# lowmee/xchu_slam

Hardware: AMD Instinct MI355X
Metric: NDT scans/sec (120k-pt scan vs 200k-voxel localmap, 30 iters) at 1/2/4/8 GPUs; % HBM BW (higher is better)
Workload: dtype f32 (f64 accumulate)

## Files before the change

### xchu_slam_amd/csrc/host_sort.hip

```cpp
#include "ndt_host.h"

namespace ndt::host {

ndt_status scan_ctx(ndt_ctx* c, Lane L, int nb, ScanCtx* sc) {
    sc->tickets = c->opt.tile_tickets ? 1 : 0;
    if ((size_t)nb > L.s.scan_status.cap) {
        TRY(ensure(c, L.s.scan_status, (size_t)nb));
        HIPCHK(c, hipMemsetAsync(L.s.scan_status.p, 0, L.s.scan_status.cap * sizeof(unsigned long long), L.st));
    }
    if (!L.s.scan_ticket.p) {
        TRY(ensure(c, L.s.scan_ticket, 1));
        HIPCHK(c, hipMemsetAsync(L.s.scan_ticket.p, 0, sizeof(unsigned long long), L.st));
        L.s.scan_tickets = 0;
    }
    sc->status = L.s.scan_status.p;
    sc->ticket = L.s.scan_ticket.p;
    sc->ticket_base = L.s.scan_tickets;
    sc->epoch = ++L.s.scan_epoch;
    sc->nb = nb;
    if (sc->tickets) L.s.scan_tickets += (unsigned long long)nb;
    return NDT_OK;
}

ndt_status enqueue_scan(ndt_ctx* c, Lane L, const int* in, int n_host, const int* n_dev, int* out, int* total_out, GridHeader* herr) {
    const int nb = std::max(1, ceil_div(n_host, kTileKeys));
    ScanCtx sc;
    TRY(scan_ctx(c, L, nb, &sc));
    hipLaunchKernelGGL(k_scan_onepass, dim3(nb), dim3(kBlock), 0, L.st, in, n_host, n_dev, out, total_out, sc, herr);
    return NDT_OK;
}

constexpr int kRadixWideKeys = 4 << 20;
int radix_items(const ndt_ctx* c, int n) {
    return ceil_div(n, kTileKeys) < c->n_cu ? 4 : (n >= kRadixWideKeys ? 24 : 16);
}
size_t radix_status_words(int nb) { return (size_t)4 * 256 * ((size_t)nb + (size_t)ceil_div(nb, 16)); }
void launch_radix_pass(const ndt_ctx* c, Lane L, int items, int nb, int* k0, int* v0, int* k1, int* v1, int n, int pass,
                       const GridHeader* h, GridHeader* herr, int last_pass) {
    auto* kern = items == 4 ? k_radix_onesweep<4> : items == 16 ? k_radix_onesweep<16> : k_radix_onesweep<24>;
    hipLaunchKernelGGL(kern, dim3(nb), dim3(kBlock), 0, L.st, k0, v0, k1, v1, n, pass, h, L.s.radix_aux.p, L.s.radix_status.p, nb,
                       herr, last_pass, c->opt.tile_tickets ? 1 : 0);
}

int radix_launch_passes(const ndt_ctx* c) {
    if (c->rerun_full) return 4;
    return c->opt.radix_force > 0 ? std::min(c->opt.radix_force, 4) : c->radix_pred;
}
void note_grid_width(ndt_ctx* c, long long cells, int dense) {
    if (cells <= 0) return;
    const long long top = dense ? cells - 1 : cells;
    int bits = 0;
    while (bits < 31 && (top >> bits) != 0) ++bits;
    c->radix_pred = std::min(4, std::max(1, (bits + 1 + 7) / 8));
}

ndt_status enqueue_bin_and_sort(ndt_ctx* c, Lane L, const float4* pts, int n, int dense, GridHeader* h, float leaf, int layout,
                                int binning, int2* cloud_span, int passes) {
    if (&L.s == &c->s && !cloud_span) c->inc_ok = false;
    const int nb_mm = std::max(1, std::min(ceil_div(n, 4 * kBlock), 1024));
    TRY(ensure(c, L.s.mm, (size_t)nb_mm * 7));
    const int items = radix_items(c, n);
    const int nb_sort = std::max(1, ceil_div(n, kBlock * items));
    const size_t n_kv = cloud_span ? (size_t)n + (size_t)n / 4 : (size_t)n;
    TRY(ensure(c, L.s.k0, n_kv)); TRY(ensure(c, L.s.v0, n_kv)); TRY(ensure(c, L.s.k1, n_kv)); TRY(ensure(c, L.s.v1, n_kv));
    TRY(ensure(c, L.s.radix_aux, kRadixAuxWords));
    TRY(ensure(c, L.s.radix_status, radix_status_words(nb_sort)));
    TRY(ensure(c, L.s.seg_start, (size_t)n + 1));
    hipLaunchKernelGGL(k_minmax, dim3(nb_mm), dim3(kBlock), 0, L.st, pts, n, dense, L.s.mm.p, L.s.radix_aux.p,
                       cloud_span ? c->d_clk.p + 3 : nullptr, nullptr, nullptr, nullptr);
    const int nb_keys = std::max(1, std::min(ceil_div(n, 4 * kBlock), 512));
    hipLaunchKernelGGL(k_keys, dim3(nb_keys), dim3(kBlock), 0, L.st, pts, n, dense, L.s.mm.p, nb_mm, h, leaf, c->prm.min_points_per_voxel,
                       c->prm.min_covar_eigvalue_mult, layout, binning, L.s.k0.p, L.s.v0.p, L.s.radix_aux.p, L.s.radix_status.p,
                       (int)radix_status_words(nb_sort), cloud_span ? c->grid.p : nullptr, (long long)c->grid.cap, cloud_span ? c->table.p : nullptr,
                       1LL << c->max_log2cap, nullptr, 0);
    for (int pass = 0; pass < passes; ++pass)
        launch_radix_pass(c, L, items, nb_sort, L.s.k0.p, L.s.v0.p, L.s.k1.p, L.s.v1.p, n, pass, h, h, passes - 1);
    const int nb_seg = std::max(1, ceil_div(n, kTileKeys));
    ScanCtx sc;
    TRY(scan_ctx(c, L, nb_seg, &sc));
    hipLaunchKernelGGL(k_seg_scan, dim3(nb_seg), dim3(kBlock), 0, L.st, L.s.k0.p, L.s.k1.p, n, h, L.s.seg_start.p, sc);
    if (cloud_span) {
        ScanCtx sc2;
        TRY(scan_ctx(c, L, nb_seg, &sc2));
        hipLaunchKernelGGL(k_cloud_scan, dim3(nb_seg), dim3(kBlock), 0, L.st, L.s.seg_start.p, n, h, cloud_span, sc2, c->max_log2cap);
    }
    return NDT_OK;
}

ndt_status enqueue_downsample_finalize(ndt_ctx* c, Lane L, const GridHeader* h, const float4* in, int n, float4* out) {
    TRY(ensure(c, L.s.sorted_pts, std::max(n, 1)));
    const int nb = std::max(1, std::min(ceil_div(n, 4 * kBlock), 2048));
    hipLaunchKernelGGL(k_sorted_gather, dim3(nb), dim3(kBlock), 0, L.st, in, L.s.v0.p, L.s.v1.p, h, L.s.sorted_pts.p, n);
    hipLaunchKernelGGL(k_downsample_finalize, dim3(std::max(1, ceil_div(n, kBlock))), dim3(kBlock), 0, L.st, L.s.sorted_pts.p,
                       L.s.seg_start.p, h, out);
    HIPCHK(c, hipGetLastError());
    return NDT_OK;
}

}
```

### xchu_slam_amd/csrc/host_target.hip

```cpp
#include "ndt_host.h"

namespace ndt::host {

namespace {

ndt_status grow_grid(ndt_ctx* c) {
    const long long want_cells = std::min<long long>(std::max<long long>(2 * c->grid_cells_seen, 16ll << 20), 1ll << 30);
    if ((long long)c->grid.cap < want_cells) TRY(ensure(c, c->grid, (size_t)want_cells));
    return NDT_OK;
}

ndt_status alloc_cloud_buffers(ndt_ctx* c, size_t max_cloud) {
    TRY(ensure(c, c->recs, max_cloud)); TRY(ensure(c, c->cent, max_cloud)); TRY(ensure(c, c->icovd, max_cloud * 9));
    TRY(ensure(c, c->evals, max_cloud * 3)); TRY(ensure(c, c->cloud_key, max_cloud));
    return NDT_OK;
}

constexpr int kFinalize3WavesMaxPoints = 4 << 20;

ndt_status prepare_target_buffers(ndt_ctx* c, int M, int* nb_cloud) {
    TRY(grow_grid(c));
    const size_t max_cloud = std::max(1, M / std::max(1, c->prm.min_points_per_voxel) + 1);
    TRY(alloc_cloud_buffers(c, max_cloud));
    unsigned l = 6;
// ... 9 lines not shown
ndt_status launch_finalize(ndt_ctx* c, int M, int nb_cloud) {
    auto* fin = M < kFinalize3WavesMaxPoints ? k_leaf_finalize<3> : k_leaf_finalize<2>;
    hipLaunchKernelGGL(fin, dim3(nb_cloud), dim3(kBlock), 0, c->stream.get(), c->target_ptr, c->s.k0.p, c->s.k1.p, c->s.v0.p,
                       c->s.v1.p, c->s.cloud_span.p, c->d_hdr.p, c->recs.p, c->cent.p, c->icovd.p, c->cloud_key.p,
                       c->evals.p, c->grid.p, c->table.p, c->valid_part.p);
    HIPCHK(c, hipGetLastError());
    return NDT_OK;
}

ndt_status enqueue_target_build(ndt_ctx* c) {
    c->inc_ok = false;
    ++c->n_builds_full;
    const int M = c->M;
    int nb_cloud = 0;
    TRY(prepare_target_buffers(c, M, &nb_cloud));
    TRY(enqueue_bin_and_sort(c, main_lane(c), c->target_ptr, M, c->target_dense, c->d_hdr.p, c->prm.resolution, 0, c->prm.precision_mode == 2 ? 1 : 0,
                             c->s.cloud_span.p, radix_launch_passes(c)));
    TRY(launch_finalize(c, M, nb_cloud));
    c->inc_ok = c->prm.precision_mode != 2 && c->target_dense == 1 && M > 0;
    return NDT_OK;
}

ndt_status enqueue_target_append(ndt_ctx* c, int n_old, int n_new, const float4* new_src) {
    const int M = n_old + n_new;
    int nb_cloud = 0;
    TRY(prepare_target_buffers(c, M, &nb_cloud));
    Lane Q{c->stream.get(), c->s_inc};
    float4* copy_to = new_src ? const_cast<float4*>(c->target_ptr) + n_old : nullptr;
    const float4* pts_new = new_src ? new_src : c->target_ptr + n_old;
    const int nq = std::max(n_new, 1);
    const int nb_mm = std::max(1, std::min(ceil_div(nq, 4 * kBlock), 1024));
    TRY(ensure(c, Q.s.mm, (size_t)nb_mm * 7));
    const int items = radix_items(c, nq);
    const int nb_sort = std::max(1, ceil_div(nq, kBlock * items));
    TRY(ensure(c, Q.s.k0, nq)); TRY(ensure(c, Q.s.v0, nq)); TRY(ensure(c, Q.s.k1, nq)); TRY(ensure(c, Q.s.v1, nq));
    TRY(ensure(c, Q.s.radix_aux, kRadixAuxWords));
    TRY(ensure(c, Q.s.radix_status, radix_status_words(nb_sort)));
    TRY(ensure(c, c->s.seg_start, (size_t)M + 1));
    hipLaunchKernelGGL(k_minmax, dim3(nb_mm), dim3(kBlock), 0, c->stream.get(), pts_new, n_new, 1, Q.s.mm.p, Q.s.radix_aux.p, c->d_clk.p + 3,
                       c->d_hdr.p, c->d_hdr_prev.p, copy_to);
    if (c->tgt_ev_valid) HIPCHK(c, hipEventRecord(c->ev_tgt.get(), c->stream.get()));
    const long long clear_words = std::max<long long>((long long)c->grid.cap, 2LL << c->max_log2cap) / 4;
    const int nb_keys = std::max(1, (int)std::min<long long>(std::max<long long>(ceil_div(nq, 4 * kBlock), ceil_div(clear_words, 4LL * kBlock)), 512));
    hipLaunchKernelGGL(k_keys, dim3(nb_keys), dim3(kBlock), 0, c->stream.get(), pts_new, n_new, 1, Q.s.mm.p, nb_mm, c->d_hdr.p, c->prm.resolution,
                       c->prm.min_points_per_voxel, c->prm.min_covar_eigvalue_mult, 0, 0, Q.s.k0.p, Q.s.v0.p, Q.s.radix_aux.p,
                       Q.s.radix_status.p, (int)radix_status_words(nb_sort), c->grid.p, (long long)c->grid.cap, c->table.p, 1LL << c->max_log2cap,
                       c->d_hdr_prev.p, n_old);
    const int passes = radix_launch_passes(c);
    for (int pass = 0; pass < passes; ++pass)
        launch_radix_pass(c, Q, items, nb_sort, Q.s.k0.p, Q.s.v0.p, Q.s.k1.p, Q.s.v1.p, n_new, pass, c->d_hdr.p, c->d_hdr.p, passes - 1);
    hipLaunchKernelGGL(k_merge_append, dim3(std::max(1, ceil_div(M, kMergeTileKeys))), dim3(kBlock), 0, c->stream.get(), c->s.k0.p, c->s.v0.p,
                       c->s.k1.p, c->s.v1.p, c->d_hdr_prev.p, n_old, Q.s.k0.p, Q.s.v0.p, Q.s.k1.p, Q.s.v1.p, n_new, c->d_hdr.p,
                       c->target_ptr);
    const Lane L = main_lane(c);
    const int nb_seg = std::max(1, ceil_div(M, kTileKeys));
    ScanCtx sc, sc2;
    TRY(scan_ctx(c, L, nb_seg, &sc));
    hipLaunchKernelGGL(k_seg_scan, dim3(nb_seg), dim3(kBlock), 0, c->stream.get(), c->s.k0.p, c->s.k1.p, M, c->d_hdr.p, c->s.seg_start.p, sc);
    TRY(scan_ctx(c, L, nb_seg, &sc2));
    hipLaunchKernelGGL(k_cloud_scan, dim3(nb_seg), dim3(kBlock), 0, c->stream.get(), c->s.seg_start.p, M, c->d_hdr.p, c->s.cloud_span.p, sc2,
                       c->max_log2cap);
    TRY(launch_finalize(c, M, nb_cloud));
    return NDT_OK;
}

}

ndt_status build_target(ndt_ctx* c) {
    ++c->tgt_gen;
    c->tgt_ev_valid = c->lanes.fit_tgt_used;
    if (c->tgt_ev_valid) HIPCHK(c, hipEventRecord(c->ev_tgt.get(), c->stream.get()));
    TRY(enqueue_target_build(c));
    c->build_unchecked = true;
    c->built_since_align = true;
    c->grid_valid = true;
    c->fit_valid = false;
    c->grid_res = c->prm.resolution;
    c->have_result = false;
    return NDT_OK;
}

ndt_status rerun_build(ndt_ctx* c, int berr) {
    ++c->n_builds_rerun;
    if (berr & kBuildErrLookback) {
        c->opt.tile_tickets = true;
        ++c->n_rerun_lookback;
    }
    c->inc_ok = false;
    c->rerun_full = true;
    const ndt_status st = build_target(c);
    c->rerun_full = false;
    return st;
}

ndt_status settle_build(ndt_ctx* c) {
    if (!c->build_unchecked || !c->grid_valid) return NDT_OK;
    for (int attempt = 0;; ++attempt) {
        HIPCHK(c, hipMemcpyAsync(c->h_hdr.get(), c->d_hdr.p, sizeof(GridHeader), hipMemcpyDeviceToHost, c->stream.get()));
        HIPCHK(c, hipStreamSynchronize(c->stream.get()));
        const int berr = c->h_hdr->pad[0];
        if (!berr) break;
        if (attempt > 0) return fail(c, NDT_EDEVICE, "target build failed twice (error bits " + std::to_string(berr) + ")");
        TRY(rerun_build(c, berr));
    }
    c->build_unchecked = false;
    note_grid_width(c, c->h_hdr->cells, c->target_dense);
    return NDT_OK;
}

ndt_status upload_points(ndt_ctx* c, DevBuf<float4>& dst, const float* xyz, size_t n, size_t stride_bytes) {
    TRY(ensure(c, dst, n));
    std::vector<float4> tmp(n);
    const char* base = reinterpret_cast<const char*>(xyz);
    for (size_t i = 0; i < n; ++i) {
// ... 165 lines not shown
```

### xchu_slam_amd/csrc/ndt_host.h

```cpp
#pragma once
#include <hip/hip_runtime.h>
#include <string>
#include <vector>
#include <cstring>
#include <cstdlib>
#include <cstdio>
#include <algorithm>
#include <cmath>
#include <atomic>
#include <condition_variable>
#include <deque>
#include <functional>
#include <memory>
#include <mutex>
#include <shared_mutex>
#include <thread>

#include "../../include/ndt_hip.h"
#include "ndt_kernels.h"
#include "ndt_geom.h"

namespace ndt::host {

constexpr int kTileKeys = kBlock * 16;
// ... 310 lines not shown

#define TRY(expr)                          \
    do {                                   \
        ndt_status _s = (expr);            \
        if (_s != NDT_OK) return _s;       \
    } while (0)

template <typename T> ndt_status make_pinned(ndt_ctx* c, Pinned<T>& out, size_t n, unsigned flags) {
    void* p = nullptr;
    if (hipHostMalloc(&p, n * sizeof(std::remove_extent_t<T>), flags) != hipSuccess) return fail(c, NDT_ENOMEM, "hipHostMalloc failed");
    out.reset(static_cast<std::remove_extent_t<T>*>(p));
    return NDT_OK;
}
inline ndt_status make_event(ndt_ctx* c, Event& out, unsigned flags) {
    hipEvent_t e = nullptr;
    HIPCHK(c, hipEventCreateWithFlags(&e, flags));
    out.reset(e);
    return NDT_OK;
}
inline ndt_status make_stream(ndt_ctx* c, Stream& out, int priority) {
    hipStream_t st = nullptr;
    HIPCHK(c, hipStreamCreateWithPriority(&st, hipStreamNonBlocking, priority));
    out.reset(st);
    return NDT_OK;
}

inline void hand_options(ndt_ctx* h, const ndt_ctx* c) {
    const bool sticky = h->opt.tile_tickets;
    h->opt = c->opt;
    h->opt.tile_tickets = sticky || c->opt.tile_tickets;
}

inline ndt_status set_dev(ndt_ctx* c) {
    HIPCHK(c, hipSetDevice(c->device));
    return NDT_OK;
}

inline ndt_status need_target_and_source(ndt_ctx* c) {
    if (!c->has_target) return fail(c, NDT_ENOTARGET, "no input target");
    if (!c->has_source || c->N == 0) return fail(c, NDT_ENOSOURCE, "no input source");
    return NDT_OK;
}

ndt_status scan_ctx(ndt_ctx* c, Lane L, int nb, ScanCtx* sc);
ndt_status enqueue_scan(ndt_ctx* c, Lane L, const int* in, int n_host, const int* n_dev, int* out, int* total_out, GridHeader* herr);
int radix_items(const ndt_ctx* c, int n);
size_t radix_status_words(int nb);
void launch_radix_pass(const ndt_ctx* c, Lane L, int items, int nb, int* k0, int* v0, int* k1, int* v1, int n, int pass,
                       const GridHeader* h, GridHeader* herr, int last_pass = 3);
int radix_launch_passes(const ndt_ctx* c);
void note_grid_width(ndt_ctx* c, long long cells, int dense);
ndt_status enqueue_bin_and_sort(ndt_ctx* c, Lane L, const float4* pts, int n, int dense, GridHeader* h, float leaf, int layout = 0,
                                int binning = 0, int2* cloud_span = nullptr, int passes = 4);
ndt_status enqueue_downsample_finalize(ndt_ctx* c, Lane L, const GridHeader* h, const float4* in, int n, float4* out);
ndt_status build_target(ndt_ctx* c);
ndt_status rerun_build(ndt_ctx* c, int berr);
ndt_status settle_build(ndt_ctx* c);
ndt_status upload_points(ndt_ctx* c, DevBuf<float4>& dst, const float* xyz, size_t n, size_t stride_bytes);
void invalidate_graph(ndt_ctx* c);
ndt_status copy16(ndt_ctx* c, hipStream_t stream, void* dst, const void* src, size_t bytes);
ndt_status flush_source(ndt_ctx* c);
ndt_status capture_graph(ndt_ctx* c, const char* end_what, const std::function<ndt_status()>& body, GraphExec* out);
ndt_status main_after_fit(ndt_ctx* c, bool source);
ndt_status enqueue_nn_index(ndt_ctx* c, Lane L, const float4* pts, int n, int dense, float cell, NNIndex& ix, bool want_idx = false);
ndt_status ensure_fit_index(ndt_ctx* c);
ndt_status voxel_downsample_dev(ndt_ctx* c, const float4* in, size_t n, float leaf, float4* out, size_t* n_out);
ndt_status reserve_slots(ndt_ctx* c, SlotArrays& a, size_t size, size_t need, std::initializer_list<size_t> slot_bytes, const char* what);

}
```

### xchu_slam_amd/csrc/ndt_kernels.h

```cpp
#pragma once
#include <hip/hip_runtime.h>
#include "ndt_types.h"
#include "ndt_linalg.h"
#include "ndt_icp.h"
#include "ndt_sc.h"
#include "ndt_isc.h"
#include "ndt_pgo.h"
#include "ndt_map.h"

namespace ndt {
__global__ void k_minmax(const float4*, int, int, float*, int*, unsigned long long*, const GridHeader*, GridHeader*, float4*);
__global__ void k_keys(const float4*, int, int, const float*, int, GridHeader*, float, int, double, int, int, int*, int*, int*, unsigned*, int,
                       int*, long long, int2*, long long, const GridHeader*, int);
__global__ void k_merge_append(int*, int*, int*, int*, const GridHeader*, int, const int*, const int*, const int*, const int*, int,
                               GridHeader*, const float4*);
template <int ITEMS>
__global__ void k_radix_onesweep(int*, int*, int*, int*, int, int, const GridHeader*, int*, unsigned*, int, GridHeader*, int, int);
__global__ void k_scan_onepass(const int*, int, const int*, int*, int*, ScanCtx, GridHeader*);
__global__ void k_seg_scan(const int*, const int*, int, GridHeader*, int*, ScanCtx);
__global__ void k_cloud_scan(const int*, int, GridHeader*, int2*, ScanCtx, unsigned);

template <int WAVES>
__global__ void k_leaf_finalize(const float4*, const int*, const int*, const int*, const int*, const int2*, GridHeader*,
                                VoxelRec*, float4*, double*, int*, double*, int*, int2*, int*);
__global__ void k_sorted_gather(const float4*, const int*, const int*, const GridHeader*, float4*, int);
__global__ void k_src_keys(const float4*, int, Mat4f, const GridHeader*, int*, int*, int*, unsigned*, int);
__global__ void k_src_gather(const float4*, const int*, const int*, const GridHeader*, float4*, int);
__global__ void k_crop_flags(const float4*, int, double, double, int*);
__global__ void k_compact4(const float4*, const int*, const int*, int, float4*);
template <int C>
__global__ void k_sor_knn(const float4*, int, int, const GridHeader*, const int*, const int*, const float4*, float*);
__global__ void k_sor_stats(const float*, int, double, double*);
__global__ void k_sor_keep(const float*, int, const double*, int*);
__global__ void k_ror_keep(const float4*, int, double, int, const GridHeader*, const int*, const int*, const float4*, int*);
__global__ void k_downsample_finalize(const float4*, const int*, const GridHeader*, float4*);
__global__ void k_fit_gather(const float4*, const int*, const int*, const int*, const int*, const int*, int, const GridHeader*, float4*,
                             int*, int*, int*);
__global__ void k_icp_pass(float4*, int, IcpState*, const GridHeader*, const int*, const int*, const float4*, const int*, int*, float*,
                           double*, unsigned*, IcpRecordDev*);
__global__ void k_sc_make(const float4*, int, unsigned*);
__global__ void k_sc_finalize(const unsigned*, ScDb, int);
__global__ void k_sc_detect(ScDb, const int*, const int*, int, int, ScDetectArgs, ndt_sc_result*);
__global__ void k_isc_make(const float4*, int, IscGeom, unsigned*);
__global__ void k_isc_finalize(const unsigned*, IscDb, int, int, int, double, double, double, double);
__global__ void k_isc_detect(IscDb, const int*, int, IscDetectArgs, IscPartial*);
__global__ void k_isc_reduce(const IscPartial*, const int*, int, int, IscDetectArgs, ndt_isc_result*);
__global__ void k_pgo_optimize(PgoGraph, PgoArgs);
__global__ void k_map_stack(const float4*, const int*, const long long*, const Mat4f*, int, int, int, float4*);
__global__ void k_fit_block_flags(const int*, const GridHeader*, int*);
__global__ void k_append2(const float4*, const float4*, int, const GridHeader*, float4*, float4*);
__global__ void k_fit_block_clear(int*, const GridHeader*);
__global__ void k_fit_tables(const int*, const int*, const int*, const int*, const GridHeader*, int*, int*);
__global__ void k_fitness(const float4*, int, Mat4f, const GridHeader*, const int*, const int*, const float4*, double, float*, double*,
                          int*, unsigned*, double*, long long*);
__global__ void k_score_radius(const float4*, int, Mat4f, const GridHeader*, const int2*, const int*, const VoxelRec*, const float4*,
                               const double*, double, double, double, float, double*);
template <int SEARCH, int PPT, bool ONE_TILE>
__global__ void k_pass_direct(const float4*, int, int, const GridHeader*, const int2*, const int*, const VoxelRec*, const AlignState*,
                              AlignState*, double*, unsigned*, double*, PassRecordDev*, int, int, unsigned long long*, int4*);
__global__ void k_pass_radius(const float4*, int, const GridHeader*, const int2*, const int*, const VoxelRec*, const float4*,
                              const double*, const AlignState*, AlignState*, double*, unsigned*, double*, PassRecordDev*, int, int,
                              unsigned long long*);
__global__ void k_transform(const float4*, int, const AlignState*, float4*);
__global__ void k_transform_mat(const float4*, int, Mat4f, float4*);
__global__ void k_align_init(const AlignState, AlignState*, unsigned*, unsigned long long*, int, unsigned long long*, const GridHeader*,
                             unsigned long long, const uint4*, uint4*, long long);
__global__ void k_copy16(const uint4*, uint4*, size_t);
__global__ void k_readback(const unsigned long long*, unsigned long long*, int, const unsigned long long*, unsigned long long*, int,
                           const unsigned long long*, unsigned long long*, int, const unsigned long long*, unsigned long long*,
                           unsigned long long*, unsigned long long, unsigned long long*, const GridHeader*);
hipError_t dbg_read_blk(unsigned long long* host, size_t count);
__global__ void k_svd_resume(AlignState*);
template <int SEARCH, bool ONE_TILE>
// ... 4 lines not shown
```

### xchu_slam_amd/csrc/voxel_build.hip

```cpp
#include "ndt_device.h"
#include "ndt_kernels.h"

namespace ndt {

constexpr int kTileItems = 16;
constexpr int kTile = kBlock * kTileItems;
constexpr int kRadixAux = kRadixAuxWords;

__global__ __launch_bounds__(kBlock) void k_minmax(const float4* __restrict__ pts, int n, int is_dense, float* __restrict__ part,
                                                   int* __restrict__ radix_aux, unsigned long long* __restrict__ clk_start,
                                                   const GridHeader* __restrict__ hdr_cur, GridHeader* __restrict__ hdr_save,
                                                   float4* __restrict__ copy_to) {
    if (clk_start && blockIdx.x == 0 && threadIdx.x == 0) *clk_start = __builtin_amdgcn_s_memrealtime();
    if (blockIdx.x == 0) {
        for (int i = threadIdx.x; i < kRadixAux; i += kBlock) radix_aux[i] = 0;
        if (hdr_save) {
            static_assert(sizeof(GridHeader) % 4 == 0 && sizeof(GridHeader) / 4 <= kBlock, "header copy: one word per thread");
            if (threadIdx.x < sizeof(GridHeader) / 4)
                reinterpret_cast<int*>(hdr_save)[threadIdx.x] = reinterpret_cast<const int*>(hdr_cur)[threadIdx.x];
        }
    }
    float mn[3] = {FLT_MAX, FLT_MAX, FLT_MAX}, mx[3] = {-FLT_MAX, -FLT_MAX, -FLT_MAX};
    int cnt = 0;
    const int stride = gridDim.x * kBlock;
// ... 483 lines not shown
__device__ __forceinline__ int scan_n(int n, const int* n_dev) { return n_dev ? *n_dev : n; }

__device__ __forceinline__ const int* sorted_buf_nominal(const GridHeader* h, const int* b0, const int* b1) {
    const int passes = (h->key_bits + 7) / 8;
    return (passes & 1) ? b1 : b0;
}
__device__ __forceinline__ const int* sorted_buf(const GridHeader* h, const int* b0, const int* b1) {
    const int passes = (h->key_bits + 7) / 8;
    return ((passes + h->flip) & 1) ? b1 : b0;
}

constexpr unsigned long long kScanAgg = 1ull << 30, kScanPre = 2ull << 30, kScanVal = (1ull << 30) - 1;

__device__ long long scan_lookback(unsigned long long* __restrict__ status, int tile, int tot, unsigned epoch,
                                   GridHeader* __restrict__ herr) {
    const int lane = threadIdx.x & 63;
    const unsigned long long tag = (unsigned long long)epoch << 32;
    if (lane == 0)
        __hip_atomic_store(&status[tile], tag | (tile == 0 ? kScanPre : kScanAgg) | (unsigned long long)tot, __ATOMIC_RELAXED,
                           __HIP_MEMORY_SCOPE_AGENT);
    long long excl = 0;
    int t = tile - 1;
    int spin = 0;
    while (t >= 0) {
        const int tt = t - lane;
        unsigned long long wd = 0;
        bool ready = true;
        if (tt >= 0) {
            wd = __hip_atomic_load(&status[tt], __ATOMIC_RELAXED, __HIP_MEMORY_SCOPE_AGENT);
            ready = (wd >> 32) == epoch && (wd & (kScanAgg | kScanPre)) != 0;
        }
        const bool pre = tt >= 0 && ready && (wd & kScanPre);
        const unsigned long long pre_mask = __ballot(pre);
        const int stop = pre_mask ? (__ffsll((long long)pre_mask) - 1) : 63;
        const unsigned long long need = (stop == 63) ? ~0ull : ((2ull << stop) - 1);
        const unsigned long long not_ready = __ballot(!ready) & need;
        if (not_ready) {
            if (++spin > kSpinLimit) { if (lane == 0) atomicOr(&herr->pad[0], kBuildErrLookback); break; }
            __builtin_amdgcn_s_sleep(1);
            continue;
        }
        long long v = (tt >= 0 && lane <= stop) ? (long long)(wd & kScanVal) : 0;
        for (int m = 32; m > 0; m >>= 1) v += __shfl_xor(v, m, 64);
        excl += v;
        if (pre_mask) break;
        t -= 64;
    }
    if (lane == 0 && tile > 0)
        __hip_atomic_store(&status[tile], tag | kScanPre | ((unsigned long long)(excl + tot) & kScanVal), __ATOMIC_RELAXED,
                           __HIP_MEMORY_SCOPE_AGENT);
    return excl;
}

__device__ __forceinline__ int tile_scan(const ScanCtx& sc, int sum, GridHeader* herr, int* s_tile, int* s_excl, int* lds, int tile,
                                         int* total) {
    int tot;
    const int ex = block_exclusive_scan(sum, lds, &tot);
    if (threadIdx.x < 64) {
        const long long excl = scan_lookback(sc.status, tile, tot, sc.epoch, herr);
        if (threadIdx.x == 0) *s_excl = (int)excl;
    }
    __syncthreads();
    *total = *s_excl + tot;
    return ex + *s_excl;
}

__device__ __forceinline__ int take_ticket(const ScanCtx& sc, int* s_tile) {
    if (threadIdx.x == 0) *s_tile = sc.tickets ? (int)(atomicAdd(sc.ticket, 1ull) - sc.ticket_base) : (int)blockIdx.x;
    __syncthreads();
    return *s_tile;
}

constexpr int kStageWords = kTile + 2 + (kTile + 2) / 32 + 1;
__host__ __device__ constexpr int st_idx(int p) { return p + (p >> 5); }
template <int EXTRA>
__device__ __forceinline__ void stage_tile(const int* __restrict__ in, long long first, int n, int fill, int* s) {
    constexpr int R = (kTile + EXTRA + kBlock - 1) / kBlock;
    int v[R];
#pragma unroll
    for (int r = 0; r < R; ++r) {
        const int p = threadIdx.x + r * kBlock;
        const long long i = first + p;
        v[r] = (p < kTile + EXTRA && i >= 0 && i < n) ? in[i] : fill;
    }
#pragma unroll
    for (int r = 0; r < R; ++r) {
        const int p = threadIdx.x + r * kBlock;
        if (p < kTile + EXTRA) s[st_idx(p)] = v[r];
    }
    __syncthreads();
}

__global__ __launch_bounds__(kBlock) void k_scan_onepass(const int* __restrict__ in, int n, const int* n_dev, int* __restrict__ out,
                                                         int* __restrict__ total_out, ScanCtx sc, GridHeader* __restrict__ herr) {
    __shared__ int s_tile, s_excl, lds[4];
    __shared__ int s_in[kStageWords];
    const int tile = take_ticket(sc, &s_tile);
    const int nn = scan_n(n, n_dev);
    const int base = tile * kTile + threadIdx.x * kTileItems;
    stage_tile<0>(in, (long long)tile * kTile, nn, 0, s_in);
    int loc[kTileItems];
    int sum = 0;
#pragma unroll
    for (int k = 0; k < kTileItems; ++k) {
        loc[k] = s_in[st_idx(threadIdx.x * kTileItems + k)];
        sum += loc[k];
    }
    int total;
    int ex = tile_scan(sc, sum, herr, &s_tile, &s_excl, lds, tile, &total);
    if (tile == sc.nb - 1 && threadIdx.x == 0 && total_out) *total_out = total;
#pragma unroll
    for (int k = 0; k < kTileItems; ++k) {
        if (base + k < nn) out[base + k] = ex;
        ex += loc[k];
    }
// ... 61 lines not shown
            const unsigned long long probed = __ballot(m < hi);
            const unsigned long long fls = __ballot(m < hi && !t);
            if (fls == 0ull) {
                lo = lo + (63 - __clzll((long long)probed)) * step + 1;
            } else {
                const int f = __ffsll((long long)fls) - 1;
                const int nlo = f == 0 ? lo : lo + (f - 1) * step + 1;
                hi = lo + f * step;
                lo = nlo;
            }
        }
        if (lane == 0) s_split[w] = lo;
    }
    __syncthreads();
    const int a0 = s_split[0], a1 = s_split[1];
    const int la = a1 - a0, b0 = d0 - a0, lb = (d1 - d0) - la;
    for (int i = threadIdx.x; i < la; i += kBlock) {
        const int v = ov[a0 + i];
        s_k[i] = remap_key(r, ok[a0 + i], v, pts, hn);
        s_v[i] = v;
    }
    for (int i = threadIdx.x; i < lb; i += kBlock) {
        s_k[la + i] = qk[b0 + i];
        s_v[la + i] = qv[b0 + i];
    }
    __syncthreads();
    const int dl = threadIdx.x * kMergeItems;
    const int tn = d1 - d0;
    if (dl >= tn) return;
    int lo = max(0, dl - lb), hi = min(dl, la);
    while (lo < hi) {
        const int mid = (lo + hi) >> 1;
        if (s_k[mid] <= s_k[la + dl - 1 - mid]) lo = mid + 1;
        else hi = mid;
    }
    int ai = lo, bi = dl - lo;
#pragma unroll
    for (int k = 0; k < kMergeItems; ++k) {
        if (dl + k >= tn) break;
        const bool take_a = ai < la && (bi >= lb || s_k[ai] <= s_k[la + bi]);
        const int src = take_a ? ai : la + bi;
        wk[d0 + dl + k] = s_k[src];
        wv[d0 + dl + k] = s_v[src];
        ai += take_a ? 1 : 0;
        bi += take_a ? 0 : 1;
    }
}

__global__ __launch_bounds__(kBlock) void k_seg_scan(const int* __restrict__ k0, const int* __restrict__ k1, int n,
                                                     GridHeader* __restrict__ h, int* __restrict__ seg_start, ScanCtx sc) {
    __shared__ int s_tile, s_excl, lds[4];
    __shared__ int s_k[kStageWords];
    const int tile = take_ticket(sc, &s_tile);
    const bool empty = h->empty != 0;
    const int* k = sorted_buf(h, k0, k1);
    const int sentinel = h->sentinel;
    const int base = tile * kTile + threadIdx.x * kTileItems;
    unsigned heads = 0;
    int sum = 0;
    if (!empty) {
        stage_tile<1>(k, (long long)tile * kTile - 1, n, 0, s_k);
        int prev = s_k[st_idx(threadIdx.x * kTileItems)];
#pragma unroll
        for (int q = 0; q < kTileItems; ++q) {
            const int i = base + q;
            if (i >= n) break;
            const int key = s_k[st_idx(threadIdx.x * kTileItems + q + 1)];
            if (key != sentinel && (i == 0 || prev != key)) { heads |= 1u << q; ++sum; }
            prev = key;
        }
    }
    int total;
    int ex = tile_scan(sc, sum, h, &s_tile, &s_excl, lds, tile, &total);
#pragma unroll
    for (int q = 0; q < kTileItems; ++q)
        if (heads & (1u << q)) seg_start[ex++] = base + q;
    if (tile == sc.nb - 1 && threadIdx.x == 0) {
        h->n_leaves = total;
        seg_start[total] = empty ? 0 : h->n_points;
    }
}

__global__ __launch_bounds__(kBlock) void k_cloud_scan(const int* __restrict__ seg_start, int n, GridHeader* __restrict__ h,
                                                       int2* __restrict__ cloud_span, ScanCtx sc, unsigned max_log2cap) {
    __shared__ int s_tile, s_excl, lds[4];
    __shared__ int s_seg[kStageWords];
    const int tile = take_ticket(sc, &s_tile);
    const int nl = h->empty ? 0 : h->n_leaves;
    const int last = nl > 0 ? (nl - 1) / kTile : 0;
    if (tile > last) return;
    const int base = tile * kTile + threadIdx.x * kTileItems;
    const int minp = h->min_points;
    unsigned fl = 0;
    int sum = 0;
    stage_tile<1>(seg_start, (long long)tile * kTile, nl + 1, 0, s_seg);
#pragma unroll
    for (int q = 0; q < kTileItems; ++q) {
        const int s = base + q;
        if (s >= nl) break;
        const int p = threadIdx.x * kTileItems + q;
        if (s_seg[st_idx(p + 1)] - s_seg[st_idx(p)] >= minp) { fl |= 1u << q; ++sum; }
    }
    int total;
    int ex = tile_scan(sc, sum, h, &s_tile, &s_excl, lds, tile, &total);
#pragma unroll
    for (int q = 0; q < kTileItems; ++q)
        if (fl & (1u << q)) {
            const int p = threadIdx.x * kTileItems + q;
            cloud_span[ex++] = make_int2(s_seg[st_idx(p)], s_seg[st_idx(p + 1)]);
        }
    if (tile == last && threadIdx.x == 0) {
        h->n_cloud = total;
        unsigned l = 6;
        while (l < max_log2cap && (1LL << l) < 4LL * (long long)total) ++l;
        h->log2cap = l;
        if (total == 0) h->empty = 1;
    }
}






constexpr int kGather = 8;
__device__ __forceinline__ bool leaf_stats(const float4* __restrict__ pts, const int* __restrict__ idx, int b, int e, int ci, int key,
                                           const GridHeader* __restrict__ h, VoxelRec* __restrict__ recs, float4* __restrict__ cent,
                                           double* __restrict__ icovd, int* __restrict__ cloud_key, double* __restrict__ evals_out) {
    const int n = e - b;
    double sum[3] = {0.0, 0.0, 0.0};
    double cov[9] = {1.0, 0.0, 0.0, 0.0, 1.0, 0.0, 0.0, 0.0, 1.0};
    float cen[3] = {0.f, 0.f, 0.f};
    int ix[kGather];
#pragma unroll
    for (int k = 0; k < kGather; ++k) ix[k] = (b + k < e) ? idx[b + k] : -1;
    for (int j0 = b; j0 < e; j0 += kGather) {
        float4 q[kGather];
#pragma unroll
        for (int k = 0; k < kGather; ++k) q[k] = ix[k] >= 0 ? pts[ix[k]] : make_float4(0.f, 0.f, 0.f, 0.f);
#pragma unroll
        for (int k = 0; k < kGather; ++k) ix[k] = (j0 + kGather + k < e) ? idx[j0 + kGather + k] : -1;
#pragma unroll
        for (int k = 0; k < kGather; ++k) {
            if (j0 + k >= e) break;
            const float4 p = q[k];
            const double pd[3] = {(double)p.x, (double)p.y, (double)p.z};
            sum[0] += pd[0]; sum[1] += pd[1]; sum[2] += pd[2];
            for (int c = 0; c < 3; ++c)
                for (int r = 0; r < 3; ++r) cov[r + 3 * c] += pd[r] * pd[c];
            cen[0] += p.x; cen[1] += p.y; cen[2] += p.z;
        }
    }
    const float nf = (float)n;
    for (int a = 0; a < 3; ++a) cen[a] /= nf;
    const double nd = (double)n;
    double mean[3];
    for (int a = 0; a < 3; ++a) mean[a] = sum[a] / nd;
    if (h->binning)
        for (int a = 0; a < 3; ++a) cen[a] = (float)mean[a];
    for (int c = 0; c < 3; ++c)
        for (int r = 0; r < 3; ++r) cov[r + 3 * c] = (cov[r + 3 * c] - 2 * (sum[r] * mean[c])) / nd + mean[r] * mean[c];
    const double f = (n - 1.0) / n;
    for (int k = 0; k < 9; ++k) cov[k] *= f;
    double ev[3], V[9];
    if (h->binning) aw_sym_eigen3(cov, ev, V);
    else sym_eigen3(cov, ev, V);
    double icov[9] = {0, 0, 0, 0, 0, 0, 0, 0, 0};
    bool rejected = false;
    if (ev[0] < 0 || ev[1] < 0 || ev[2] <= 0) {
        rejected = true;
// ... 448 lines not shown
        s_cnt[threadIdx.x] = k;
        __syncthreads();
        for (int off = kFitBlock / 2; off > 0; off >>= 1) {
            if ((int)threadIdx.x < off) { s_sum[threadIdx.x] += s_sum[threadIdx.x + off]; s_cnt[threadIdx.x] += s_cnt[threadIdx.x + off]; }
            __syncthreads();
        }
    };
    tree(sum, cnt);
    const int nb = gridDim.x;
    const int g = blockIdx.x / kFitGroup, ng = (nb + kFitGroup - 1) / kFitGroup;
    const int g0 = g * kFitGroup, gsize = min(kFitGroup, nb - g0);
    if (threadIdx.x == 0) {
        __hip_atomic_store(part_sum + blockIdx.x, s_sum[0], __ATOMIC_RELAXED, __HIP_MEMORY_SCOPE_AGENT);
        __hip_atomic_store(part_cnt + blockIdx.x, (int)s_cnt[0], __ATOMIC_RELAXED, __HIP_MEMORY_SCOPE_AGENT);
        asm volatile("s_waitcnt vmcnt(0)" ::: "memory");
        s_role = __hip_atomic_fetch_add(&ticket[kFitTicketStride * (1 + g)], 1u, __ATOMIC_RELAXED, __HIP_MEMORY_SCOPE_AGENT) ==
                 (unsigned)gsize - 1;
    }
    __syncthreads();
    if (!s_role) return;
    __builtin_amdgcn_fence(__ATOMIC_ACQUIRE, "agent");
    asm volatile("s_waitcnt vmcnt(0)" ::: "memory");
    {
        const int t = threadIdx.x;
        tree(t < gsize ? part_sum[g0 + t] : 0.0, t < gsize ? (long long)part_cnt[g0 + t] : 0ll);
    }
    if (threadIdx.x == 0) {
        ticket[kFitTicketStride * (1 + g)] = 0u;
        __hip_atomic_store(part_sum + nb + g, s_sum[0], __ATOMIC_RELAXED, __HIP_MEMORY_SCOPE_AGENT);
        __hip_atomic_store(part_cnt + nb + g, (int)s_cnt[0], __ATOMIC_RELAXED, __HIP_MEMORY_SCOPE_AGENT);
        asm volatile("s_waitcnt vmcnt(0)" ::: "memory");
        s_role = __hip_atomic_fetch_add(&ticket[0], 1u, __ATOMIC_RELAXED, __HIP_MEMORY_SCOPE_AGENT) == (unsigned)ng - 1 ? 2 : 0;
    }
    __syncthreads();
    if (s_role != 2) return;
    __builtin_amdgcn_fence(__ATOMIC_ACQUIRE, "agent");
    asm volatile("s_waitcnt vmcnt(0)" ::: "memory");
    {
        double v = 0.0;
        long long k = 0;
        for (int t = threadIdx.x; t < ng; t += kFitBlock) { v += part_sum[nb + t]; k += part_cnt[nb + t]; }
        tree(v, k);
    }
    if (threadIdx.x == 0) {
        __hip_atomic_store(out_sum, s_sum[0], __ATOMIC_RELAXED, __HIP_MEMORY_SCOPE_SYSTEM);
        __hip_atomic_store(out_cnt, h->pad[0] ? -1ll : (long long)s_cnt[0], __ATOMIC_RELAXED, __HIP_MEMORY_SCOPE_SYSTEM);
        ticket[0] = 0u;
    }
}


}

#ifdef NDT_SORT_STAMPS
extern "C" int ndt_dbg_read_sort(unsigned long long* host, size_t count, int clear) {
    const size_t n = count < sizeof(ndt::g_sort_ts) / sizeof(unsigned long long) ? count : sizeof(ndt::g_sort_ts) / sizeof(unsigned long long);
    hipError_t e = hipDeviceSynchronize();
    if (e == hipSuccess && host) e = hipMemcpyFromSymbol(host, HIP_SYMBOL(ndt::g_sort_ts), n * sizeof(unsigned long long), 0, hipMemcpyDeviceToHost);
    if (e == hipSuccess && clear) {
        void* p = nullptr;
        e = hipGetSymbolAddress(&p, HIP_SYMBOL(ndt::g_sort_ts));
        if (e == hipSuccess) e = hipMemset(p, 0, sizeof(ndt::g_sort_ts));
    }
    return (int)e;
}
#endif
```

Measured before the change: 1305.

## Fuse segment and cloud scans into one kernel with two-level grouped look-back

Adds a fused k_seg_cloud_scan kernel that computes voxel segment heads and qualifying cloud spans in a single pass over sorted keys. It decides whether a voxel has enough points by looking ahead and back min_points keys instead of reading seg_start in a second kernel. Both counts are packed into one 32-bit look-back word, and a grouped two-level decoupled look-back replaces the serial chained look-back for mid-sized grids. This removes one kernel launch, one scan-status setup and the reread of seg_start. The cost is a more complex scan with a 16-bit packing limit per tile, bounds checks on cloud capacity, and a fallback path when min_points exceeds 8. Optional timestamp instrumentation is added behind a macro.

Result: no change. 1313, median of 6 (+0.7%).

```diff
diff --git a/xchu_slam_amd/csrc/host_sort.hip b/xchu_slam_amd/csrc/host_sort.hip
--- a/xchu_slam_amd/csrc/host_sort.hip
+++ b/xchu_slam_amd/csrc/host_sort.hip
@@ -1,11 +1,13 @@
 #include "ndt_host.h"
+#include <climits>
 
 namespace ndt::host {
 
 ndt_status scan_ctx(ndt_ctx* c, Lane L, int nb, ScanCtx* sc) {
     sc->tickets = c->opt.tile_tickets ? 1 : 0;
-    if ((size_t)nb > L.s.scan_status.cap) {
-        TRY(ensure(c, L.s.scan_status, (size_t)nb));
+    const size_t words = (size_t)scan_status_words(nb, kScanMaxCounts);
+    if (words > L.s.scan_status.cap) {
+        TRY(ensure(c, L.s.scan_status, words));
         HIPCHK(c, hipMemsetAsync(L.s.scan_status.p, 0, L.s.scan_status.cap * sizeof(unsigned long long), L.st));
     }
     if (!L.s.scan_ticket.p) {
@@ -75,9 +77,19 @@
                        1LL << c->max_log2cap, nullptr, 0);
     for (int pass = 0; pass < passes; ++pass)
         launch_radix_pass(c, L, items, nb_sort, L.s.k0.p, L.s.v0.p, L.s.k1.p, L.s.v1.p, n, pass, h, h, passes - 1);
+    return enqueue_segments(c, L, n, h, cloud_span);
+}
+
+ndt_status enqueue_segments(ndt_ctx* c, Lane L, int n, GridHeader* h, int2* cloud_span) {
     const int nb_seg = std::max(1, ceil_div(n, kTileKeys));
     ScanCtx sc;
     TRY(scan_ctx(c, L, nb_seg, &sc));
+    if (cloud_span && cloud_span == L.s.cloud_span.p && scan_fused_stage(nb_seg) && cloud_fused_minp(c->prm.min_points_per_voxel)) {
+        const int cloud_cap = (int)std::min<size_t>(L.s.cloud_span.cap, (size_t)INT_MAX);
+        hipLaunchKernelGGL(k_seg_cloud_scan, dim3(nb_seg), dim3(kBlock), 0, L.st, L.s.k0.p, L.s.k1.p, n, h, L.s.seg_start.p, cloud_span, cloud_cap,
+                           sc, c->max_log2cap);
+        return NDT_OK;
+    }
     hipLaunchKernelGGL(k_seg_scan, dim3(nb_seg), dim3(kBlock), 0, L.st, L.s.k0.p, L.s.k1.p, n, h, L.s.seg_start.p, sc);
     if (cloud_span) {
         ScanCtx sc2;
diff --git a/xchu_slam_amd/csrc/host_target.hip b/xchu_slam_amd/csrc/host_target.hip
--- a/xchu_slam_amd/csrc/host_target.hip
+++ b/xchu_slam_amd/csrc/host_target.hip
@@ -85,14 +85,7 @@
     hipLaunchKernelGGL(k_merge_append, dim3(std::max(1, ceil_div(M, kMergeTileKeys))), dim3(kBlock), 0, c->stream.get(), c->s.k0.p, c->s.v0.p,
                        c->s.k1.p, c->s.v1.p, c->d_hdr_prev.p, n_old, Q.s.k0.p, Q.s.v0.p, Q.s.k1.p, Q.s.v1.p, n_new, c->d_hdr.p,
                        c->target_ptr);
-    const Lane L = main_lane(c);
-    const int nb_seg = std::max(1, ceil_div(M, kTileKeys));
-    ScanCtx sc, sc2;
-    TRY(scan_ctx(c, L, nb_seg, &sc));
-    hipLaunchKernelGGL(k_seg_scan, dim3(nb_seg), dim3(kBlock), 0, c->stream.get(), c->s.k0.p, c->s.k1.p, M, c->d_hdr.p, c->s.seg_start.p, sc);
-    TRY(scan_ctx(c, L, nb_seg, &sc2));
-    hipLaunchKernelGGL(k_cloud_scan, dim3(nb_seg), dim3(kBlock), 0, c->stream.get(), c->s.seg_start.p, M, c->d_hdr.p, c->s.cloud_span.p, sc2,
-                       c->max_log2cap);
+    TRY(enqueue_segments(c, main_lane(c), M, c->d_hdr.p, c->s.cloud_span.p));
     TRY(launch_finalize(c, M, nb_cloud));
     return NDT_OK;
 }
diff --git a/xchu_slam_amd/csrc/ndt_host.h b/xchu_slam_amd/csrc/ndt_host.h
--- a/xchu_slam_amd/csrc/ndt_host.h
+++ b/xchu_slam_amd/csrc/ndt_host.h
@@ -386,6 +386,7 @@
 void note_grid_width(ndt_ctx* c, long long cells, int dense);
 ndt_status enqueue_bin_and_sort(ndt_ctx* c, Lane L, const float4* pts, int n, int dense, GridHeader* h, float leaf, int layout = 0,
                                 int binning = 0, int2* cloud_span = nullptr, int passes = 4);
+ndt_status enqueue_segments(ndt_ctx* c, Lane L, int n, GridHeader* h, int2* cloud_span);
 ndt_status enqueue_downsample_finalize(ndt_ctx* c, Lane L, const GridHeader* h, const float4* in, int n, float4* out);
 ndt_status build_target(ndt_ctx* c);
 ndt_status rerun_build(ndt_ctx* c, int berr);
diff --git a/xchu_slam_amd/csrc/ndt_kernels.h b/xchu_slam_amd/csrc/ndt_kernels.h
--- a/xchu_slam_amd/csrc/ndt_kernels.h
+++ b/xchu_slam_amd/csrc/ndt_kernels.h
@@ -1,6 +1,7 @@
 #pragma once
 #include <hip/hip_runtime.h>
 #include "ndt_types.h"
+#include "ndt_scan.h"
 #include "ndt_linalg.h"
 #include "ndt_icp.h"
 #include "ndt_sc.h"
@@ -19,6 +20,7 @@
 __global__ void k_scan_onepass(const int*, int, const int*, int*, int*, ScanCtx, GridHeader*);
 __global__ void k_seg_scan(const int*, const int*, int, GridHeader*, int*, ScanCtx);
 __global__ void k_cloud_scan(const int*, int, GridHeader*, int2*, ScanCtx, unsigned);
+__global__ void k_seg_cloud_scan(const int*, const int*, int, GridHeader*, int*, int2*, int, ScanCtx, unsigned);
 
 template <int WAVES>
 __global__ void k_leaf_finalize(const float4*, const int*, const int*, const int*, const int*, const int2*, GridHeader*,
diff --git a/xchu_slam_amd/csrc/ndt_scan.h b/xchu_slam_amd/csrc/ndt_scan.h
--- /dev/null
+++ b/xchu_slam_amd/csrc/ndt_scan.h
@@ -0,0 +1,69 @@
+#pragma once
+#ifndef __host__
+#define __host__
+#define __device__
+#endif
+
+namespace ndt {
+
+constexpr int kScanGroupTiles = 16;
+constexpr int kScanMaxCounts = 2;
+constexpr int kScanResidentTiles = 1024;
+constexpr int kScanChainedTiles = 128;
+#ifdef NDT_SCAN_PARENT
+constexpr int kScanTwoLevelTiles = 0;
+#else
+constexpr int kScanTwoLevelTiles = kScanResidentTiles;
+#endif
+#if defined(NDT_SCAN_PARENT) || defined(NDT_SCAN_TWO_KERNELS)
+constexpr bool kScanFusedStage = false;
+#else
+constexpr bool kScanFusedStage = true;
+#endif
+constexpr int kScanMaxGroups = kScanResidentTiles / kScanGroupTiles;
+constexpr int kScanMaxWords = kScanGroupTiles - 1 + (kScanMaxGroups - 1) * kScanMaxCounts;
+constexpr int kScanRounds = (kScanMaxWords + 63) / 64;
+
+__host__ __device__ constexpr bool scan_two_level(int nb) { return nb > kScanChainedTiles && nb <= kScanTwoLevelTiles; }
+__host__ __device__ constexpr bool scan_fused_stage(int nb) { return kScanFusedStage && nb <= kScanResidentTiles; }
+__host__ __device__ constexpr int scan_groups(int nb) { return (nb + kScanGroupTiles - 1) / kScanGroupTiles; }
+__host__ __device__ constexpr int scan_group_of(int tile) { return tile / kScanGroupTiles; }
+__host__ __device__ constexpr int scan_pos_in_group(int tile) { return tile % kScanGroupTiles; }
+__host__ __device__ constexpr bool scan_closes_group(int tile) { return scan_pos_in_group(tile) == kScanGroupTiles - 1; }
+__host__ __device__ constexpr int scan_total_index(int nb, int g, int W, int w) { return nb + g * W + w; }
+__host__ __device__ constexpr long long scan_status_words(int nb, int W) { return (long long)nb + (long long)scan_groups(nb) * W; }
+__host__ __device__ constexpr int scan_lookback_words(int tile, int W) { return scan_pos_in_group(tile) + scan_group_of(tile) * W; }
+__host__ __device__ constexpr bool scan_word_is_aggregate(int tile, int j) { return j < scan_pos_in_group(tile); }
+__host__ __device__ constexpr int scan_word_component(int tile, int W, int j) { return (j - scan_pos_in_group(tile)) % W; }
+__host__ __device__ constexpr int scan_lookback_index(int nb, int tile, int W, int j) {
+    return scan_word_is_aggregate(tile, j) ? scan_group_of(tile) * kScanGroupTiles + j
+                                           : scan_total_index(nb, (j - scan_pos_in_group(tile)) / W, W, scan_word_component(tile, W, j));
+}
+
+constexpr int kScanPackShift = 16;
+__host__ __device__ constexpr unsigned scan_pack(int a, int b) { return (unsigned)a | ((unsigned)b << kScanPackShift); }
+__host__ __device__ constexpr int scan_unpack(unsigned v, int w) { return (int)(w == 0 ? v & ((1u << kScanPackShift) - 1u) : v >> kScanPackShift); }
+
+constexpr int kCloudLookMax = 8;
+__host__ __device__ constexpr bool cloud_fused_minp(int minp) { return minp <= kCloudLookMax; }
+__host__ __device__ constexpr int cloud_look(int minp) { return minp > 1 ? minp : 1; }
+template <class I>
+__host__ __device__ constexpr bool cloud_head_test(int key, int key_ahead, I i, int look, I n) {
+    return i + look - 1 < n && key_ahead == key;
+}
+template <class I>
+__host__ __device__ constexpr bool cloud_end_test(int key_last, int key_back, I j, int look) {
+    return j >= look && key_back == key_last;
+}
+template <class KeyAt>
+__host__ __device__ inline bool cloud_head_flag(KeyAt key_at, long long i, int minp, long long n) {
+    const int look = cloud_look(minp);
+    return cloud_head_test<long long>(key_at(i), i + look - 1 < n ? key_at(i + look - 1) : 0, i, look, n);
+}
+template <class KeyAt>
+__host__ __device__ inline bool cloud_end_flag(KeyAt key_at, long long j, int minp) {
+    const int look = cloud_look(minp);
+    return cloud_end_test<long long>(key_at(j - 1), j >= look ? key_at(j - look) : 0, j, look);
+}
+
+}
diff --git a/xchu_slam_amd/csrc/voxel_build.hip b/xchu_slam_amd/csrc/voxel_build.hip
--- a/xchu_slam_amd/csrc/voxel_build.hip
+++ b/xchu_slam_amd/csrc/voxel_build.hip
@@ -559,15 +559,118 @@
     return excl;
 }
 
+template <int W>
+__device__ __forceinline__ bool scan_lookback_two_level(unsigned long long* __restrict__ status, int nb, int tile, const int (&tot)[W],
+                                                        unsigned epoch, GridHeader* __restrict__ herr, int (&excl)[W]) {
+    static_assert(W >= 1 && W <= kScanMaxCounts, "counts per look-back");
+    const int lane = threadIdx.x & 63;
+    const unsigned long long tag = (unsigned long long)epoch << 32;
+    const unsigned mine = W == 2 ? scan_pack(tot[0], tot[W - 1]) : (unsigned)tot[0];
+    if (lane == 0) __hip_atomic_store(&status[tile], tag | kScanAgg | (unsigned long long)mine, __ATOMIC_RELAXED, __HIP_MEMORY_SCOPE_AGENT);
+    const int p = scan_pos_in_group(tile), g = scan_group_of(tile);
+    const int m = scan_lookback_words(tile, W);
+    bool closed = !scan_closes_group(tile);
+    int spin = 0;
+    for (int w = 0; w < W; ++w) excl[w] = 0;
+    while (m > 0) {
+        unsigned long long wd[kScanRounds];
+#pragma unroll
+        for (int r = 0; r < kScanRounds; ++r) {
+            const int j = lane + 64 * r;
+            wd[r] = j < m ? __hip_atomic_load(&status[scan_lookback_index(nb, tile, W, j)], __ATOMIC_RELAXED, __HIP_MEMORY_SCOPE_AGENT) : 0ull;
+        }
+        bool ready = true, ready0 = true;
+        int v[W];
+        for (int w = 0; w < W; ++w) v[w] = 0;
+#pragma unroll
+        for (int r = 0; r < kScanRounds; ++r) {
+            const int j = lane + 64 * r;
+            if (j >= m) continue;
+            ready = ready && (wd[r] >> 32) == epoch && (wd[r] & kScanAgg) != 0;
+            if (r == 0) ready0 = ready;
+            const unsigned val = (unsigned)(wd[r] & kScanVal);
+            if (scan_word_is_aggregate(tile, j)) {
+                for (int w = 0; w < W; ++w) v[w] += W == 2 ? scan_unpack(val, w) : (int)val;
+            } else {
+                const int comp = scan_word_component(tile, W, j);
+                for (int w = 0; w < W; ++w) v[w] += w == comp ? (int)val : 0;
+            }
+        }
+        if (!closed && __ballot(lane < p && !ready0) == 0ull) {
+            for (int w = 0; w < W; ++w) {
+                int s = lane < p ? (W == 2 ? scan_unpack((unsigned)(wd[0] & kScanVal), w) : (int)(wd[0] & kScanVal)) : 0;
+                for (int k = 32; k > 0; k >>= 1) s += __shfl_xor(s, k, 64);
+                if (lane == 0)
+                    __hip_atomic_store(&status[scan_total_index(nb, g, W, w)], tag | kScanAgg | ((unsigned long long)(s + tot[w]) & kScanVal),
+                                       __ATOMIC_RELAXED, __HIP_MEMORY_SCOPE_AGENT);
+            }
+            closed = true;
+        }
+        if (__ballot(!ready) == 0ull) {
+            for (int w = 0; w < W; ++w) {
+                int s = v[w];
+                for (int k = 32; k > 0; k >>= 1) s += __shfl_xor(s, k, 64);
+                excl[w] = s;
+            }
+            return true;
+        }
+        if (++spin > kSpinLimit) { if (lane == 0) atomicOr(&herr->pad[0], kBuildErrLookback); return false; }
+        __builtin_amdgcn_s_sleep(1);
+    }
+    return true;
+}
+
+#ifdef NDT_SCAN_STAMPS
+constexpr int kScanStampWords = 16;
+__device__ unsigned long long g_scan_ts[3 * 3 * kScanStampWords];
+struct ScanStamp {
+    unsigned long long* row;
+    unsigned long long t0;
+};
+__device__ __forceinline__ ScanStamp scan_stamp_begin(int kid, int tile, int nb) {
+    const int cls = tile == 0 ? 0 : tile == nb - 1 ? 2 : tile == nb / 2 ? 1 : -1;
+    ScanStamp s{threadIdx.x == 0 && cls >= 0 ? &g_scan_ts[(kid * 3 + cls) * kScanStampWords] : nullptr, __builtin_amdgcn_s_memrealtime()};
+    if (s.row) { s.row[0] += 1ull; s.row[6] = (unsigned long long)nb; s.row[8] = s.t0; }
+    return s;
+}
+__device__ __forceinline__ void scan_stamp(const ScanStamp& s, int slot) {
+    __syncthreads();
+    if (s.row) {
+        const unsigned long long now = __builtin_amdgcn_s_memrealtime();
+        s.row[slot] += now - s.t0;
+        s.row[8 + slot] = now;
+    }
+}
+#define NDT_SCAN_STAMP_BEGIN(kid, nb) const ScanStamp scan_st = scan_stamp_begin(kid, tile, nb)
+#define NDT_SCAN_STAMP(slot) scan_stamp(scan_st, slot)
+#define NDT_SCAN_STAMP_PARAM , ScanStamp scan_st = ScanStamp{nullptr, 0ull}
+#define NDT_SCAN_STAMP_ARG , scan_st
+#else
+#define NDT_SCAN_STAMP_BEGIN(kid, nb) do { } while (0)
+#define NDT_SCAN_STAMP(slot) do { } while (0)
+#define NDT_SCAN_STAMP_PARAM
+#define NDT_SCAN_STAMP_ARG
+#endif
+
 __device__ __forceinline__ int tile_scan(const ScanCtx& sc, int sum, GridHeader* herr, int* s_tile, int* s_excl, int* lds, int tile,
-                                         int* total) {
+                                         int* total NDT_SCAN_STAMP_PARAM) {
     int tot;
     const int ex = block_exclusive_scan(sum, lds, &tot);
+    NDT_SCAN_STAMP(2);
     if (threadIdx.x < 64) {
-        const long long excl = scan_lookback(sc.status, tile, tot, sc.epoch, herr);
+        long long excl;
+        if (scan_two_level(sc.nb)) {
+            const int t1[1] = {tot};
+            int e1[1];
+            scan_lookback_two_level<1>(sc.status, sc.nb, tile, t1, sc.epoch, herr, e1);
+            excl = e1[0];
+        } else {
+            excl = scan_lookback(sc.status, tile, tot, sc.epoch, herr);
+        }
         if (threadIdx.x == 0) *s_excl = (int)excl;
     }
     __syncthreads();
+    NDT_SCAN_STAMP(3);
     *total = *s_excl + tot;
     return ex + *s_excl;
 }
@@ -735,6 +838,7 @@
     __shared__ int s_tile, s_excl, lds[4];
     __shared__ int s_k[kStageWords];
     const int tile = take_ticket(sc, &s_tile);
+    NDT_SCAN_STAMP_BEGIN(0, sc.nb);
     const bool empty = h->empty != 0;
     const int* k = sorted_buf(h, k0, k1);
     const int sentinel = h->sentinel;
@@ -753,8 +857,9 @@
             prev = key;
         }
     }
+    NDT_SCAN_STAMP(1);
     int total;
-    int ex = tile_scan(sc, sum, h, &s_tile, &s_excl, lds, tile, &total);
+    int ex = tile_scan(sc, sum, h, &s_tile, &s_excl, lds, tile, &total NDT_SCAN_STAMP_ARG);
 #pragma unroll
     for (int q = 0; q < kTileItems; ++q)
         if (heads & (1u << q)) seg_start[ex++] = base + q;
@@ -762,6 +867,7 @@
         h->n_leaves = total;
         seg_start[total] = empty ? 0 : h->n_points;
     }
+    NDT_SCAN_STAMP(4);
 }
 
 __global__ __launch_bounds__(kBlock) void k_cloud_scan(const int* __restrict__ seg_start, int n, GridHeader* __restrict__ h,
@@ -772,6 +878,7 @@
     const int nl = h->empty ? 0 : h->n_leaves;
     const int last = nl > 0 ? (nl - 1) / kTile : 0;
     if (tile > last) return;
+    NDT_SCAN_STAMP_BEGIN(1, last + 1);
     const int base = tile * kTile + threadIdx.x * kTileItems;
     const int minp = h->min_points;
     unsigned fl = 0;
@@ -784,8 +891,9 @@
         const int p = threadIdx.x * kTileItems + q;
         if (s_seg[st_idx(p + 1)] - s_seg[st_idx(p)] >= minp) { fl |= 1u << q; ++sum; }
     }
+    NDT_SCAN_STAMP(1);
     int total;
-    int ex = tile_scan(sc, sum, h, &s_tile, &s_excl, lds, tile, &total);
+    int ex = tile_scan(sc, sum, h, &s_tile, &s_excl, lds, tile, &total NDT_SCAN_STAMP_ARG);
 #pragma unroll
     for (int q = 0; q < kTileItems; ++q)
         if (fl & (1u << q)) {
@@ -799,6 +907,91 @@
         h->log2cap = l;
         if (total == 0) h->empty = 1;
     }
+    NDT_SCAN_STAMP(4);
+}
+
+constexpr int kCloudStageExtra = kCloudLookMax + kCloudLookMax - 1;
+constexpr int kCloudStageWords = st_idx(kTile + kCloudStageExtra) + 1;
+__global__ __launch_bounds__(kBlock) void k_seg_cloud_scan(const int* __restrict__ k0, const int* __restrict__ k1, int n,
+                                                           GridHeader* __restrict__ h, int* __restrict__ seg_start,
+                                                           int2* __restrict__ cloud_span, int cloud_cap, ScanCtx sc,
+                                                           unsigned max_log2cap) {
+    __shared__ int s_tile, s_excl[3], lds[4];
+    __shared__ int s_k[kCloudStageWords];
+    const int tile = take_ticket(sc, &s_tile);
+    NDT_SCAN_STAMP_BEGIN(2, sc.nb);
+    const bool empty = h->empty != 0 || h->pad[0] != 0;
+    const int* k = sorted_buf(h, k0, k1);
+    const int sentinel = h->sentinel;
+    const int minp = h->min_points;
+    const int base = tile * kTile + threadIdx.x * kTileItems;
+    unsigned heads = 0, clouds = 0, ends = 0;
+    bool last_end = false;
+    int sum = 0;
+    if (!empty) {
+        stage_tile<kCloudStageExtra>(k, (long long)tile * kTile - kCloudLookMax, n, sentinel, s_k);
+        const int look = min(cloud_look(minp), kCloudLookMax);
+        const int l0 = threadIdx.x * kTileItems + kCloudLookMax;
+        int prev = s_k[st_idx(l0 - 1)];
+#pragma unroll
+        for (int q = 0; q < kTileItems; ++q) {
+            const int i = base + q;
+            const int key = s_k[st_idx(l0 + q)];
+            const int back = s_k[st_idx(l0 + q - look)];
+            const int ahead = s_k[st_idx(l0 + q + look - 1)];
+            const bool bound = i < n && (i == 0 || prev != key);
+            const bool head = bound && key != sentinel;
+            const bool cloud = head && cloud_head_test(key, ahead, i, look, n);
+            const bool end = bound && i > 0 && prev != sentinel && cloud_end_test(prev, back, i, look);
+            heads |= (head ? 1u : 0u) << q;
+            clouds |= (cloud ? 1u : 0u) << q;
+            ends |= (end ? 1u : 0u) << q;
+            sum += (head ? 1 : 0) + (cloud ? 1 << kScanPackShift : 0);
+            if (i == n - 1 && key != sentinel && cloud_end_test(key, s_k[st_idx(l0 + q + 1 - look)], n, look)) last_end = true;
+            prev = key;
+        }
+    }
+    NDT_SCAN_STAMP(1);
+    int tot;
+    const int exl = block_exclusive_scan(sum, lds, &tot);
+    NDT_SCAN_STAMP(2);
+    if (threadIdx.x < 64) {
+        const int t2[2] = {scan_unpack((unsigned)tot, 0), scan_unpack((unsigned)tot, 1)};
+        int e2[2];
+        const bool ok = scan_lookback_two_level<2>(sc.status, sc.nb, tile, t2, sc.epoch, h, e2);
+        if (threadIdx.x == 0) {
+            s_excl[0] = e2[0];
+            s_excl[1] = e2[1];
+            s_excl[2] = ok ? 0 : 1;
+            if (!ok) { h->n_cloud = 0; h->empty = 1; }
+        }
+    }
+    __syncthreads();
+    NDT_SCAN_STAMP(3);
+    if (s_excl[2]) { heads = clouds = ends = 0u; last_end = false; }
+    int ex = s_excl[0] + scan_unpack((unsigned)exl, 0), cex = s_excl[1] + scan_unpack((unsigned)exl, 1);
+    int* span = reinterpret_cast<int*>(cloud_span);
+#pragma unroll
+    for (int q = 0; q < kTileItems; ++q) {
+        if ((ends & (1u << q)) && cex > 0 && cex <= cloud_cap) span[2 * (cex - 1) + 1] = base + q;
+        if (heads & (1u << q)) seg_start[ex++] = base + q;
+        if (clouds & (1u << q)) {
+            if (cex < cloud_cap) span[2 * cex] = base + q;
+            ++cex;
+        }
+    }
+    if (last_end && cex > 0 && cex <= cloud_cap) span[2 * (cex - 1) + 1] = n;
+    if (tile == sc.nb - 1 && threadIdx.x == 0) {
+        const int total = s_excl[0] + scan_unpack((unsigned)tot, 0), ctotal = min(s_excl[1] + scan_unpack((unsigned)tot, 1), cloud_cap);
+        h->n_leaves = total;
+        seg_start[total] = empty ? 0 : h->n_points;
+        h->n_cloud = h->pad[0] ? 0 : ctotal;
+        unsigned l = 6;
+        while (l < max_log2cap && (1LL << l) < 4LL * (long long)ctotal) ++l;
+        h->log2cap = l;
+        if (ctotal == 0 || h->pad[0]) h->empty = 1;
+    }
+    NDT_SCAN_STAMP(4);
 }
 
 
@@ -1353,6 +1546,20 @@
 
 }
 
+#ifdef NDT_SCAN_STAMPS
+extern "C" int ndt_dbg_read_scan(unsigned long long* host, size_t count, int clear) {
+    const size_t n = count < sizeof(ndt::g_scan_ts) / sizeof(unsigned long long) ? count : sizeof(ndt::g_scan_ts) / sizeof(unsigned long long);
+    hipError_t e = hipDeviceSynchronize();
+    if (e == hipSuccess && host) e = hipMemcpyFromSymbol(host, HIP_SYMBOL(ndt::g_scan_ts), n * sizeof(unsigned long long), 0, hipMemcpyDeviceToHost);
+    if (e == hipSuccess && clear) {
+        void* p = nullptr;
+        e = hipGetSymbolAddress(&p, HIP_SYMBOL(ndt::g_scan_ts));
+        if (e == hipSuccess) e = hipMemset(p, 0, sizeof(ndt::g_scan_ts));
+    }
+    return (int)e;
+}
+#endif
+
 #ifdef NDT_SORT_STAMPS
 extern "C" int ndt_dbg_read_sort(unsigned long long* host, size_t count, int clear) {
     const size_t n = count < sizeof(ndt::g_sort_ts) / sizeof(unsigned long long) ? count : sizeof(ndt::g_sort_ts) / sizeof(unsigned long long);
```
